# stwerner97/model-based-pde-control

Measured on AMD Instinct MI355X. Metric: KS sub-steps/sec (batched env), higher is better.
Workload: dtype f64

## Files before the change

model-based-pde-control_amd/csrc/fno.hip:

```cpp
#include <hip/hip_runtime.h>

#include <cstdio>
#include <map>
#include <mutex>
#include <utility>

#include "../../include/spectral/forward_select.h"
#include "../../include/spectral_hip.h"
#include "capi_error.h"

namespace {

typedef float f32x4 __attribute__((ext_vector_type(4)));

constexpr int C = 32;
constexpr int M = 16;
constexpr int K2 = 2 * M;
constexpr int KP = K2 + 4;
constexpr int KS = 2;
constexpr int TPB = 512;
constexpr int LAYERS = 4;

struct Weights {
    const float* lift_w;
// ... 27 lines not shown
    float cscale, cshift;
};

struct BwdArgs {
    Weights w;
    Rows u, act;
    const float* gdelta;
    const float* gout;
    int gout_t;
    const float* pre;
    float* gspec;
    float* rows;
    float* dbase;
    float* dact;
    const float* tabg;
    int n, nb, pairs;
    int spec_pairs, spec_pair0;
    float cscale;
};

constexpr int R_LIFT_W = 0, R_LIFT_B = 64, R_LAYER = 96, R_LAYER_SZ = 1024 + 32;
constexpr int R_P1W = R_LAYER + LAYERS * R_LAYER_SZ, R_P1B = R_P1W + 1024, R_P2W = R_P1B + 32, R_P2B = R_P2W + 32;
constexpr int ROW = ((R_P2B + 1 + 63) / 64) * 64;

__device__ __forceinline__ void gelu_parts(float x, float& cdf, float& pdf) {
    const float ax = fabsf(x);
    const float e = __expf(-0.5f * x * x);
    const float t = __frcp_rn(fmaf(0.3275911f * 0.70710678118654752f, ax, 1.0f));
    float poly = fmaf(1.061405429f, t, -1.453152027f);
    poly = fmaf(poly, t, 1.421413741f);
    poly = fmaf(poly, t, -0.284496736f);
    poly = fmaf(poly, t, 0.254829592f);
    const float erf_abs = fmaf(-poly * t, e, 1.0f);
    cdf = 0.5f * (1.0f + copysignf(erf_abs, x));
    pdf = 0.3989422804014327f * e;
}
__device__ __forceinline__ float gelu(float x) {
    float cdf, pdf;
    gelu_parts(x, cdf, pdf);
    return x * cdf;
}
__device__ __forceinline__ float gelu_grad(float x) {
    float cdf, pdf;
    gelu_parts(x, cdf, pdf);
    return fmaf(x, pdf, cdf);
}

#ifdef FNO_STAMP
__device__ unsigned long long g_stamps[256];
#define STAMP(k)                                                                      \
    do {                                                                              \
        if (blockIdx.x == 0 && threadIdx.x == 0) g_stamps[(k)] = __builtin_amdgcn_s_memtime(); \
    } while (0)
#else
#define STAMP(k) do { } while (0)
#endif

struct Lds {
    float *xs, *tb, *S, *Z, *wps, *gv, *misc;
    int NP;
    __device__ Lds(float* base, int N) {
        NP = N + 4;
        xs = base;
        tb = xs + C * NP;
        S = tb + C * NP;
        Z = S + KS * C * KP;
        wps = Z + C * KP;
        gv = wps + C * KP;
        misc = gv + N;
    }
    static size_t floats(int N) { return 2 * (size_t)C * (N + 4) + (KS + 2) * C * KP + (size_t)N + 256; }
};

__global__ void twiddle_init_kernel(float* tab, int N) {
    const int i = blockIdx.x * blockDim.x + threadIdx.x;
    if (i >= K2 * N) return;
    const int k = i / N, n = i - k * N;
    const bool is_sin = k >= M;
    const int mode = is_sin ? k - M : k;
    const int idx = (int)(((long)mode * n) % N);
    const float ang = 2.0f * (float)idx / (float)N;
    tab[i] = is_sin ? -sinpif(ang) : cospif(ang);
}
__device__ __forceinline__ void load_table(float* tab, const float* __restrict__ tabg, int N, int NP) {
    const int sh = __ffs(N) - 1;
    for (int i = threadIdx.x; i < (K2 * N) >> 2; i += blockDim.x) {
        const int e = i << 2, k = e >> sh, n = e & (N - 1);
        *reinterpret_cast<float4*>(tab + k * NP + n) = reinterpret_cast<const float4*>(tabg)[i];
    }
}

__device__ __forceinline__ void contract_n(const float* arows, const float* brows, float* S, int N, int NP) {
    const int lane = threadIdx.x & 63, wave = threadIdx.x >> 6, nwaves = blockDim.x >> 6;
    const int r = lane & 15, q = lane >> 4;
    for (int t = wave; t < 4 * KS; t += nwaves) {
        const int tile = t & 3, ks = t >> 2, rt = tile >> 1, ct = tile & 1;
        const int span = N / KS, kbeg = ks * span;
        const float* arow = arows + (16 * rt + r) * NP + kbeg;
        const float* brow = brows + (16 * ct + r) * NP + kbeg;
        f32x4 acc0 = {0.f, 0.f, 0.f, 0.f}, acc1 = {0.f, 0.f, 0.f, 0.f}, acc2 = {0.f, 0.f, 0.f, 0.f}, acc3 = {0.f, 0.f, 0.f, 0.f};
        for (int k0 = 0; k0 < span; k0 += 16) {
            const float a0 = arow[k0 + q], a1 = arow[k0 + 4 + q], a2 = arow[k0 + 8 + q], a3 = arow[k0 + 12 + q];
            const float b0 = brow[k0 + q], b1 = brow[k0 + 4 + q], b2 = brow[k0 + 8 + q], b3 = brow[k0 + 12 + q];
            acc0 = __builtin_amdgcn_mfma_f32_16x16x4f32(a0, b0, acc0, 0, 0, 0);
            acc1 = __builtin_amdgcn_mfma_f32_16x16x4f32(a1, b1, acc1, 0, 0, 0);
            acc2 = __builtin_amdgcn_mfma_f32_16x16x4f32(a2, b2, acc2, 0, 0, 0);
            acc3 = __builtin_amdgcn_mfma_f32_16x16x4f32(a3, b3, acc3, 0, 0, 0);
        }
        float* dst = S + ks * C * KP;
#pragma unroll
        for (int j = 0; j < 4; ++j) dst[(16 * rt + 4 * q + j) * KP + 16 * ct + r] = (acc0[j] + acc1[j]) + (acc2[j] + acc3[j]);
    }
}

__device__ __forceinline__ float s_sum(const float* S, int idx) {
    float v = S[idx];
#pragma unroll
    for (int ks = 1; ks < KS; ++ks) v += S[ks * C * KP + idx];
    return v;
}

__device__ __forceinline__ void load_mat(float* dst, const float* src) {
    for (int i = threadIdx.x; i < C * C; i += blockDim.x) dst[(i >> 5) * KP + (i & 31)] = src[i];
}

__device__ __forceinline__ void lift_into(float* xs, const float* u, const float* act, const Weights& w, int N, int NP) {
    const int sh = __ffs(N) - 1;
    for (int i = threadIdx.x; i < C * N; i += blockDim.x) {
        const int c = i >> sh, n = i & (N - 1);
        xs[c * NP + n] = fmaf(w.lift_w[2 * c], u[n], fmaf(w.lift_w[2 * c + 1], act[n], w.lift_b[c]));
    }
}

struct MixRegs {
    float4 vr[8], vi[8];
};
template <bool CONJ>
__device__ __forceinline__ void mix_load(const float* __restrict__ wr, const float* __restrict__ wi, MixRegs& m) {
    const int t = threadIdx.x, q4 = t & 3, m4 = (t >> 2) & 3, row = t >> 4;
#pragma unroll
    for (int c8 = 0; c8 < 8; ++c8) {
        const int c = 8 * q4 + c8;
        const size_t widx = CONJ ? ((size_t)row * C + c) * M + 4 * m4 : ((size_t)c * C + row) * M + 4 * m4;
        m.vr[c8] = *reinterpret_cast<const float4*>(wr + widx);
        m.vi[c8] = *reinterpret_cast<const float4*>(wi + widx);
    }
}
template <bool CONJ>
__device__ __forceinline__ void mix_compute(const MixRegs& w, const float* in, float* out, float s0, float s1) {
    const int t = threadIdx.x, q4 = t & 3, m4 = (t >> 2) & 3, row = t >> 4;
    float yr[4] = {0.f, 0.f, 0.f, 0.f}, yi[4] = {0.f, 0.f, 0.f, 0.f};
#pragma unroll
    for (int c8 = 0; c8 < 8; ++c8) {
        const int c = 8 * q4 + c8;
        float xr[4], xi[4];
#pragma unroll
        for (int j = 0; j < 4; ++j) {
            const int m = 4 * m4 + j;
            xr[j] = CONJ ? in[c * KP + m] : s_sum(in, c * KP + m);
            xi[j] = CONJ ? in[c * KP + M + m] : s_sum(in, c * KP + M + m);
        }
        const float wrv[4] = {w.vr[c8].x, w.vr[c8].y, w.vr[c8].z, w.vr[c8].w};
        const float wiv[4] = {w.vi[c8].x, w.vi[c8].y, w.vi[c8].z, w.vi[c8].w};
#pragma unroll
        for (int j = 0; j < 4; ++j) {
            if (CONJ) {
                yr[j] = fmaf(xr[j], wrv[j], fmaf(xi[j], wiv[j], yr[j]));
                yi[j] = fmaf(xi[j], wrv[j], fmaf(-xr[j], wiv[j], yi[j]));
            } else {
                yr[j] = fmaf(xr[j], wrv[j], fmaf(-xi[j], wiv[j], yr[j]));
                yi[j] = fmaf(xr[j], wiv[j], fmaf(xi[j], wrv[j], yi[j]));
            }
        }
    }
#pragma unroll
    for (int j = 0; j < 4; ++j) {
        yr[j] += __shfl_xor(yr[j], 1, 64);
        yi[j] += __shfl_xor(yi[j], 1, 64);
        yr[j] += __shfl_xor(yr[j], 2, 64);
        yi[j] += __shfl_xor(yi[j], 2, 64);
    }
    if (q4 == 0) {
#pragma unroll
        for (int j = 0; j < 4; ++j) {
            const int m = 4 * m4 + j;
            const float s = m == 0 ? s0 : s1;
            out[row * KP + m] = s * yr[j];
            out[row * KP + M + m] = s * yi[j];
        }
    }
}

template <bool SAVE>
__global__ void __launch_bounds__(TPB) fno_forward_kernel(const FwdArgs a) {
    extern __shared__ __align__(16) float lds_raw[];
    const int N = a.n;
    const Lds L(lds_raw, N);
    const int NP = L.NP;
    const int p = blockIdx.x, t = p / a.nb, b = p - t * a.nb;
    const int lane = threadIdx.x & 63, wave = threadIdx.x >> 6, nwaves = blockDim.x >> 6;
    const int r = lane & 15, q = lane >> 4;
    const float* u = a.u.row(t, b);
    const float* act = a.act.row(t, b);

    STAMP(0);
    lift_into(L.xs, u, act, a.w, N, NP);
    STAMP(1);
    load_table(L.tb, a.tabg, N, NP);
    __syncthreads();
    STAMP(2);

    const float s0 = 1.0f / (float)N, s1 = 2.0f / (float)N;
    for (int l = 0; l < LAYERS; ++l) {
        STAMP(3 + 4 * l);
        MixRegs mw;
        mix_load<false>(a.w.wr[l], a.w.wi[l], mw);
        contract_n(L.xs, L.tb, L.S, N, NP);
        load_mat(L.wps, a.w.pw[l]);
        if (threadIdx.x < C) L.misc[threadIdx.x] = a.w.pb[l][threadIdx.x];
        __syncthreads();
        STAMP(4 + 4 * l);
        if (SAVE) {
            for (int i = threadIdx.x; i < C * K2; i += blockDim.x) {
                const int k = i >> 5, c = i & 31;
                a.xspec[(((size_t)l * K2 + k) * a.spec_pairs + a.spec_pair0 + p) * C + c] = s_sum(L.S, c * KP + k);
            }
        }
        mix_compute<false>(mw, L.S, L.Z, s0, s1);
        __syncthreads();
        STAMP(5 + 4 * l);
        float* pre_out = SAVE ? a.pre + ((size_t)p * LAYERS + l) * C * N : nullptr;
        for (int ct = wave; ct < (N >> 4); ct += nwaves) {
            const int pos = 16 * ct + r;
            f32x4 acc[2][2];
#pragma unroll
            for (int rt = 0; rt < 2; ++rt) {
                acc[rt][0] = f32x4{0.f, 0.f, 0.f, 0.f};
                acc[rt][1] = f32x4{0.f, 0.f, 0.f, 0.f};
                const float* zrow = L.Z + (16 * rt + r) * KP;
                const float* wrow = L.wps + (16 * rt + r) * KP;
#pragma unroll
                for (int k0 = 0; k0 < K2; k0 += 4) {
                    acc[rt][0] = __builtin_amdgcn_mfma_f32_16x16x4f32(zrow[k0 + q], L.tb[(k0 + q) * NP + pos], acc[rt][0], 0, 0, 0);
                    acc[rt][1] = __builtin_amdgcn_mfma_f32_16x16x4f32(wrow[k0 + q], L.xs[(k0 + q) * NP + pos], acc[rt][1], 0, 0, 0);
                }
            }
#pragma unroll
            for (int rt = 0; rt < 2; ++rt)
#pragma unroll
                for (int j = 0; j < 4; ++j) {
                    const int row = 16 * rt + 4 * q + j;
                    const float v = (acc[rt][0][j] + acc[rt][1][j]) + L.misc[row];
                    if (SAVE) pre_out[(size_t)row * N + pos] = v;
                    L.xs[row * NP + pos] = l + 1 < LAYERS ? gelu(v) : v;
                }
        }
        __syncthreads();
        STAMP(6 + 4 * l);
    }

    STAMP(19);
    load_mat(L.wps, a.w.p1_w);
    if (threadIdx.x < C) {
        L.misc[threadIdx.x] = a.w.p1_b[threadIdx.x];
        L.misc[C + threadIdx.x] = a.w.p2_w[threadIdx.x];
    }
    __syncthreads();
    const float b2 = a.w.p2_b[0];
    for (int ct = wave; ct < (N >> 4); ct += nwaves) {
        const int pos = 16 * ct + r;
        float part = 0.0f;
#pragma unroll
        for (int rt = 0; rt < 2; ++rt) {
            f32x4 acc = {0.f, 0.f, 0.f, 0.f};
            const float* wrow = L.wps + (16 * rt + r) * KP;
#pragma unroll
            for (int k0 = 0; k0 < C; k0 += 4)
                acc = __builtin_amdgcn_mfma_f32_16x16x4f32(wrow[k0 + q], L.xs[(k0 + q) * NP + pos], acc, 0, 0, 0);
#pragma unroll
            for (int j = 0; j < 4; ++j) {
                const int row = 16 * rt + 4 * q + j;
                part = fmaf(L.misc[C + row], gelu(acc[j] + L.misc[row]), part);
            }
        }
        part += __shfl_xor(part, 16, 64);
        part += __shfl_xor(part, 32, 64);
        if (q == 0) {
            const float d = part + b2;
            a.delta[(size_t)p * N + pos] = d;
            if (a.out) a.out[(size_t)p * N + pos] = fmaf(a.cscale, d, u[pos]) + a.cshift;
        }
    }
    STAMP(20);
}

struct SelectArgs {
    Weights w[FNO_MAX_MEMBERS];
    float cscale[FNO_MAX_MEMBERS], cshift[FNO_MAX_MEMBERS];
    const int* chosen;
    const int* step;
    const float* u;
    const float* act;
    float* out;
    const float* tabg;
    int members, T, n, nb;
};

__global__ void __launch_bounds__(TPB) fno_forward_select_kernel(const SelectArgs a) {
    extern __shared__ __align__(16) float lds_raw[];
    const int N = a.n;
    const int b = blockIdx.x;
    const int t = a.step ? __builtin_amdgcn_readfirstlane(a.step[0]) : 0;
    if (t < 0 || t >= a.T) return;
    const int pick = a.chosen ? __builtin_amdgcn_readfirstlane(a.chosen[(long)t * a.nb + b]) : 0;
    float* out = a.out + (size_t)b * N;
    if (pick < 0 || pick >= a.members) {
        for (int n = threadIdx.x; n < N; n += blockDim.x) out[n] = NAN;
        return;
    }
    const Weights& w = a.w[pick];
    const float cscale = a.cscale[pick], cshift = a.cshift[pick];
    const Lds L(lds_raw, N);
    const int NP = L.NP;
    const int lane = threadIdx.x & 63, wave = threadIdx.x >> 6, nwaves = blockDim.x >> 6;
    const int r = lane & 15, q = lane >> 4;
    const float* u = a.u + (size_t)b * N;
    const float* act = a.act + (size_t)b * N;

    lift_into(L.xs, u, act, w, N, NP);
    load_table(L.tb, a.tabg, N, NP);
    __syncthreads();

    const float s0 = 1.0f / (float)N, s1 = 2.0f / (float)N;
    for (int l = 0; l < LAYERS; ++l) {
        MixRegs mw;
        mix_load<false>(w.wr[l], w.wi[l], mw);
        contract_n(L.xs, L.tb, L.S, N, NP);
        load_mat(L.wps, w.pw[l]);
        if (threadIdx.x < C) L.misc[threadIdx.x] = w.pb[l][threadIdx.x];
        __syncthreads();
        mix_compute<false>(mw, L.S, L.Z, s0, s1);
        __syncthreads();
        for (int ct = wave; ct < (N >> 4); ct += nwaves) {
            const int pos = 16 * ct + r;
            f32x4 acc[2][2];
#pragma unroll
            for (int rt = 0; rt < 2; ++rt) {
                acc[rt][0] = f32x4{0.f, 0.f, 0.f, 0.f};
                acc[rt][1] = f32x4{0.f, 0.f, 0.f, 0.f};
                const float* zrow = L.Z + (16 * rt + r) * KP;
                const float* wrow = L.wps + (16 * rt + r) * KP;
#pragma unroll
                for (int k0 = 0; k0 < K2; k0 += 4) {
                    acc[rt][0] = __builtin_amdgcn_mfma_f32_16x16x4f32(zrow[k0 + q], L.tb[(k0 + q) * NP + pos], acc[rt][0], 0, 0, 0);
                    acc[rt][1] = __builtin_amdgcn_mfma_f32_16x16x4f32(wrow[k0 + q], L.xs[(k0 + q) * NP + pos], acc[rt][1], 0, 0, 0);
                }
            }
#pragma unroll
            for (int rt = 0; rt < 2; ++rt)
#pragma unroll
                for (int j = 0; j < 4; ++j) {
                    const int row = 16 * rt + 4 * q + j;
                    const float v = (acc[rt][0][j] + acc[rt][1][j]) + L.misc[row];
                    L.xs[row * NP + pos] = l + 1 < LAYERS ? gelu(v) : v;
                }
        }
        __syncthreads();
    }

    load_mat(L.wps, w.p1_w);
    if (threadIdx.x < C) {
        L.misc[threadIdx.x] = w.p1_b[threadIdx.x];
        L.misc[C + threadIdx.x] = w.p2_w[threadIdx.x];
    }
    __syncthreads();
    const float b2 = w.p2_b[0];
    for (int ct = wave; ct < (N >> 4); ct += nwaves) {
        const int pos = 16 * ct + r;
        float part = 0.0f;
#pragma unroll
        for (int rt = 0; rt < 2; ++rt) {
            f32x4 acc = {0.f, 0.f, 0.f, 0.f};
            const float* wrow = L.wps + (16 * rt + r) * KP;
#pragma unroll
            for (int k0 = 0; k0 < C; k0 += 4)
                acc = __builtin_amdgcn_mfma_f32_16x16x4f32(wrow[k0 + q], L.xs[(k0 + q) * NP + pos], acc, 0, 0, 0);
#pragma unroll
            for (int j = 0; j < 4; ++j) {
                const int row = 16 * rt + 4 * q + j;
                part = fmaf(L.misc[C + row], gelu(acc[j] + L.misc[row]), part);
            }
        }
        part += __shfl_xor(part, 16, 64);
        part += __shfl_xor(part, 32, 64);
        if (q == 0) {
            const float d = part + b2;
            out[pos] = fmaf(cscale, d, u[pos]) + cshift;
        }
    }
}

__device__ __forceinline__ float row_dot(const float* buf, const float* v, int N, int NP) {
    const int row = threadIdx.x >> 4, l16 = threadIdx.x & 15;
    float s = 0.0f;
    if (row < C) {
        const float* src = buf + row * NP;
        if (v) {
            for (int n = l16; n < N; n += 16) s = fmaf(src[n], v[n], s);
        } else {
            for (int n = l16; n < N; n += 16) s += src[n];
        }
    }
    s += __shfl_xor(s, 1, 64);
    s += __shfl_xor(s, 2, 64);
    s += __shfl_xor(s, 4, 64);
    s += __shfl_xor(s, 8, 64);
    return s;
}

__global__ void __launch_bounds__(TPB) fno_backward_kernel(const BwdArgs a) {
    extern __shared__ __align__(16) float lds_raw[];
    const int N = a.n;
    const Lds L(lds_raw, N);
    const int NP = L.NP;
    float* db = L.tb;
    const int p = blockIdx.x, t = p / a.nb, b = p - t * a.nb;
    const int lane = threadIdx.x & 63, wave = threadIdx.x >> 6, nwaves = blockDim.x >> 6;
    const int r = lane & 15, q = lane >> 4;
    const int sh = __ffs(N) - 1;
    const float* u = a.u.row(t, b);
    const float* act = a.act.row(t, b);
    float* grow = a.rows + (size_t)p * ROW;
    const float* pre_p = a.pre + (size_t)p * LAYERS * C * N;
    const bool has_gout = a.gout && t == a.gout_t;

    for (int n = threadIdx.x; n < N; n += blockDim.x) {
        float g = a.gdelta[(size_t)p * N + n];
        if (has_gout) g = fmaf(a.cscale, a.gout[(size_t)b * N + n], g);
        L.gv[n] = g;
    }
    {
        const float4* src = reinterpret_cast<const float4*>(pre_p + (size_t)(LAYERS - 1) * C * N);
        for (int i = threadIdx.x; i < (C * N) >> 2; i += blockDim.x) {
            const int e = i << 2, c = e >> sh, n = e & (N - 1);
            *reinterpret_cast<float4*>(L.xs + c * NP + n) = src[i];
        }
    }
    load_mat(L.wps, a.w.p1_w);
    if (threadIdx.x < C) {
        L.misc[threadIdx.x] = a.w.p1_b[threadIdx.x];
        L.misc[C + threadIdx.x] = a.w.p2_w[threadIdx.x];
    }
    __syncthreads();

    {
        float dw2[2][4] = {{0.f, 0.f, 0.f, 0.f}, {0.f, 0.f, 0.f, 0.f}};
        for (int ct = wave; ct < (N >> 4); ct += nwaves) {
            const int pos = 16 * ct + r;
            const float g = L.gv[pos];
#pragma unroll
            for (int rt = 0; rt < 2; ++rt) {
                f32x4 acc = {0.f, 0.f, 0.f, 0.f};
                const float* wrow = L.wps + (16 * rt + r) * KP;
#pragma unroll
                for (int k0 = 0; k0 < C; k0 += 4)
                    acc = __builtin_amdgcn_mfma_f32_16x16x4f32(wrow[k0 + q], L.xs[(k0 + q) * NP + pos], acc, 0, 0, 0);
#pragma unroll
                for (int j = 0; j < 4; ++j) {
                    const int row = 16 * rt + 4 * q + j;
                    const float z1 = acc[j] + L.misc[row];
                    dw2[rt][j] = fmaf(g, gelu(z1), dw2[rt][j]);
                    db[row * NP + pos] = L.misc[C + row] * g * gelu_grad(z1);
                }
            }
        }
#pragma unroll
        for (int rt = 0; rt < 2; ++rt)
#pragma unroll
            for (int j = 0; j < 4; ++j) {
                float v = dw2[rt][j];
                v += __shfl_xor(v, 1, 64);
                v += __shfl_xor(v, 2, 64);
                v += __shfl_xor(v, 4, 64);
                v += __shfl_xor(v, 8, 64);
                if (r == 0) L.Z[wave * C + 16 * rt + 4 * q + j] = v;
            }
    }
    __syncthreads();
    contract_n(db, L.xs, L.S, N, NP);
    {
        const float s = row_dot(db, nullptr, N, NP);
        if ((threadIdx.x & 15) == 0 && (threadIdx.x >> 4) < C) grow[R_P1B + (threadIdx.x >> 4)] = s;
        if (threadIdx.x < C) {
            float v = L.Z[threadIdx.x];
            for (int w = 1; w < TPB / 64; ++w) v += L.Z[w * C + threadIdx.x];
            grow[R_P2W + threadIdx.x] = v;
        }
        if (wave == 0) {
            float g = 0.0f;
            for (int n = lane; n < N; n += 64) g += L.gv[n];
#pragma unroll
            for (int m = 1; m < 64; m <<= 1) g += __shfl_xor(g, m, 64);
            if (lane == 0) grow[R_P2B] = g;
        }
    }
    __syncthreads();
    for (int i = threadIdx.x; i < C * C; i += blockDim.x) grow[R_P1W + i] = s_sum(L.S, (i >> 5) * KP + (i & 31));
    for (int ct = wave; ct < (N >> 4); ct += nwaves) {
        const int pos = 16 * ct + r;
        f32x4 acc[2];
#pragma unroll
        for (int rt = 0; rt < 2; ++rt) {
            acc[rt] = f32x4{0.f, 0.f, 0.f, 0.f};
#pragma unroll
            for (int k0 = 0; k0 < C; k0 += 4)
                acc[rt] = __builtin_amdgcn_mfma_f32_16x16x4f32(L.wps[(k0 + q) * KP + 16 * rt + r], db[(k0 + q) * NP + pos], acc[rt], 0, 0, 0);
        }
#pragma unroll
        for (int rt = 0; rt < 2; ++rt)
#pragma unroll
            for (int j = 0; j < 4; ++j) db[(16 * rt + 4 * q + j) * NP + pos] = acc[rt][j];
    }
    __syncthreads();

    const float s0 = 1.0f / (float)N, s1 = 2.0f / (float)N;
    for (int l = LAYERS - 1; l >= 0; --l) {
        if (l + 1 < LAYERS) {
            const float4* src = reinterpret_cast<const float4*>(pre_p + (size_t)l * C * N);
            for (int i = threadIdx.x; i < (C * N) >> 2; i += blockDim.x) {
                const int e = i << 2, c = e >> sh, n = e & (N - 1);
                const float4 v = src[i];
                float4* d = reinterpret_cast<float4*>(db + c * NP + n);
                float4 g = *d;
                g.x *= gelu_grad(v.x);
                g.y *= gelu_grad(v.y);
                g.z *= gelu_grad(v.z);
                g.w *= gelu_grad(v.w);
                *d = g;
            }
        }
        if (l > 0) {
            const float4* src = reinterpret_cast<const float4*>(pre_p + (size_t)(l - 1) * C * N);
            for (int i = threadIdx.x; i < (C * N) >> 2; i += blockDim.x) {
                const int e = i << 2, c = e >> sh, n = e & (N - 1);
                float4 v = src[i];
                v.x = gelu(v.x);
                v.y = gelu(v.y);
                v.z = gelu(v.z);
                v.w = gelu(v.w);
                *reinterpret_cast<float4*>(L.xs + c * NP + n) = v;
            }
        } else {
            lift_into(L.xs, u, act, a.w, N, NP);
        }
        load_mat(L.wps, a.w.pw[l]);
        __syncthreads();
        contract_n(db, L.xs, L.S, N, NP);
        {
            const float s = row_dot(db, nullptr, N, NP);
            if ((threadIdx.x & 15) == 0 && (threadIdx.x >> 4) < C) grow[R_LAYER + l * R_LAYER_SZ + 1024 + (threadIdx.x >> 4)] = s;
        }
        __syncthreads();
        for (int i = threadIdx.x; i < C * C; i += blockDim.x)
            grow[R_LAYER + l * R_LAYER_SZ + i] = s_sum(L.S, (i >> 5) * KP + (i & 31));
        load_table(L.xs, a.tabg, N, NP);
        __syncthreads();
        MixRegs mw;
        mix_load<true>(a.w.wr[l], a.w.wi[l], mw);
        contract_n(db, L.xs, L.S, N, NP);
        __syncthreads();
        for (int i = threadIdx.x; i < C * K2; i += blockDim.x) {
            const int k = i >> 5, c = i & 31, m = k & (M - 1);
            const float g = s_sum(L.S, c * KP + k) * (m == 0 ? s0 : s1);
            L.Z[c * KP + k] = g;
            a.gspec[(((size_t)l * K2 + k) * a.spec_pairs + a.spec_pair0 + p) * C + c] = g;
        }
        __syncthreads();
        mix_compute<true>(mw, L.Z, L.S, 1.0f, 1.0f);
        __syncthreads();
        for (int ct = wave; ct < (N >> 4); ct += nwaves) {
            const int pos = 16 * ct + r;
            f32x4 acc[2][2];
#pragma unroll
            for (int rt = 0; rt < 2; ++rt) {
                acc[rt][0] = f32x4{0.f, 0.f, 0.f, 0.f};
                acc[rt][1] = f32x4{0.f, 0.f, 0.f, 0.f};
                const float* zrow = L.S + (16 * rt + r) * KP;
#pragma unroll
                for (int k0 = 0; k0 < K2; k0 += 4) {
                    acc[rt][0] = __builtin_amdgcn_mfma_f32_16x16x4f32(zrow[k0 + q], L.xs[(k0 + q) * NP + pos], acc[rt][0], 0, 0, 0);
                    acc[rt][1] = __builtin_amdgcn_mfma_f32_16x16x4f32(L.wps[(k0 + q) * KP + 16 * rt + r], db[(k0 + q) * NP + pos], acc[rt][1], 0, 0, 0);
                }
            }
#pragma unroll
            for (int rt = 0; rt < 2; ++rt)
#pragma unroll
                for (int j = 0; j < 4; ++j) db[(16 * rt + 4 * q + j) * NP + pos] = acc[rt][0][j] + acc[rt][1][j];
        }
        __syncthreads();
    }

    for (int n = threadIdx.x; n < N; n += blockDim.x) {
        L.gv[n] = u[n];
        L.Z[n] = act[n];
    }
    if (threadIdx.x < C) {
        L.misc[threadIdx.x] = a.w.lift_w[2 * threadIdx.x];
        L.misc[C + threadIdx.x] = a.w.lift_w[2 * threadIdx.x + 1];
    }
    __syncthreads();
    {
        const float su = row_dot(db, L.gv, N, NP), sa = row_dot(db, L.Z, N, NP), sb = row_dot(db, nullptr, N, NP);
        if ((threadIdx.x & 15) == 0 && (threadIdx.x >> 4) < C) {
            const int c = threadIdx.x >> 4;
            grow[R_LIFT_W + 2 * c] = su;
            grow[R_LIFT_W + 2 * c + 1] = sa;
            grow[R_LIFT_B + c] = sb;
        }
    }
    if (a.dbase) {
        for (int n = threadIdx.x; n < N; n += blockDim.x) {
            float s = 0.0f;
#pragma unroll 8
            for (int c = 0; c < C; ++c) s = fmaf(L.misc[c], db[c * NP + n], s);
            if (has_gout) s += a.gout[(size_t)b * N + n];
            a.dbase[(size_t)p * N + n] = s;
        }
    }
    if (a.dact) {
        for (int n = threadIdx.x; n < N; n += blockDim.x) {
            float s = 0.0f;
#pragma unroll 8
            for (int c = 0; c < C; ++c) s = fmaf(L.misc[C + c], db[c * NP + n], s);
            a.dact[(size_t)p * N + n] = s;
        }
    }
}

__global__ void __launch_bounds__(512) fno_reduce_rows_kernel(const float* rows, int pairs, int width, float* out) {
    __shared__ float part[8][64];
    const int col = threadIdx.x & 63, grp = threadIdx.x >> 6;
    const int j = blockIdx.x * 64 + col;
    float s0 = 0.0f, s1 = 0.0f, s2 = 0.0f, s3 = 0.0f;
    if (j < width) {
        int p = grp;
        for (; p + 24 < pairs; p += 32) {
            s0 += rows[(size_t)p * width + j];
            s1 += rows[(size_t)(p + 8) * width + j];
            s2 += rows[(size_t)(p + 16) * width + j];
            s3 += rows[(size_t)(p + 24) * width + j];
        }
        for (; p < pairs; p += 8) s0 += rows[(size_t)p * width + j];
    }
    part[grp][col] = (s0 + s1) + (s2 + s3);
    __syncthreads();
    if (grp == 0 && j < width) {
        float v = part[0][col];
#pragma unroll
        for (int g = 1; g < 8; ++g) v += part[g][col];
        out[j] = v;
    }
}

struct WgradOut {
    float* dwr[LAYERS];
    float* dwi[LAYERS];
};

constexpr int WG_KS = 4;
__global__ void __launch_bounds__(256 * WG_KS) fno_spec_wgrad_kernel(const float* xspec, const float* gspec, int pairs, const WgradOut dst) {
    __shared__ float part[WG_KS][4][2][256];
    const int l = blockIdx.x / M, m = blockIdx.x % M;
    const int lane = threadIdx.x & 63, wave = threadIdx.x >> 6;
    const int tile = wave & 3, ks = wave >> 2;
    const int r = lane & 15, q = lane >> 4;
    const int rt = tile >> 1, ct = tile & 1;
    const size_t plane = (size_t)pairs * C;
    const float* xr = xspec + ((size_t)l * K2 + m) * plane;
    const float* xi = xspec + ((size_t)l * K2 + M + m) * plane;
    const float* gr = gspec + ((size_t)l * K2 + m) * plane;
    const float* gi = gspec + ((size_t)l * K2 + M + m) * plane;
    f32x4 rr = {0.f, 0.f, 0.f, 0.f}, ii = {0.f, 0.f, 0.f, 0.f}, ir = {0.f, 0.f, 0.f, 0.f}, ri = {0.f, 0.f, 0.f, 0.f};
    for (int p0 = 4 * ks; p0 < pairs; p0 += 4 * WG_KS) {
        const int pp = p0 + q;
        const bool ok = pp < pairs;
        const size_t row = (size_t)(ok ? pp : 0) * C;
        const float axr = ok ? xr[row + 16 * rt + r] : 0.f, axi = ok ? xi[row + 16 * rt + r] : 0.f;
        const float bgr = ok ? gr[row + 16 * ct + r] : 0.f, bgi = ok ? gi[row + 16 * ct + r] : 0.f;
        rr = __builtin_amdgcn_mfma_f32_16x16x4f32(axr, bgr, rr, 0, 0, 0);
        ii = __builtin_amdgcn_mfma_f32_16x16x4f32(axi, bgi, ii, 0, 0, 0);
        ir = __builtin_amdgcn_mfma_f32_16x16x4f32(axr, bgi, ir, 0, 0, 0);
        ri = __builtin_amdgcn_mfma_f32_16x16x4f32(axi, bgr, ri, 0, 0, 0);
    }
#pragma unroll
    for (int j = 0; j < 4; ++j) {
        part[ks][tile][0][lane * 4 + j] = rr[j] + ii[j];
        part[ks][tile][1][lane * 4 + j] = ir[j] - ri[j];
    }
    __syncthreads();
    if (ks == 0) {
        float* outr = dst.dwr[l];
        float* outi = dst.dwi[l];
#pragma unroll
        for (int j = 0; j < 4; ++j) {
            float vr = part[0][tile][0][lane * 4 + j], vi = part[0][tile][1][lane * 4 + j];
#pragma unroll
            for (int k = 1; k < WG_KS; ++k) {
                vr += part[k][tile][0][lane * 4 + j];
                vi += part[k][tile][1][lane * 4 + j];
            }
            const int i = 16 * rt + 4 * q + j, o = 16 * ct + r;
            const size_t idx = ((size_t)i * C + o) * M + m;
            outr[idx] = vr;
            outi[idx] = vi;
        }
    }
}

int check(const char* who, int n, int nb, int pairs, int width, int modes, int layers) {
// ... 200 lines not shown
```

Before: 1.366 billion.

## Restructure FNO kernels with register-held MFMA tiles, software-pipelined contraction, prefetched loads

After: 1.363 billion. Within noise of the previous version (-0.2%).

```diff
diff --git a/model-based-pde-control_amd/csrc/fno.hip b/model-based-pde-control_amd/csrc/fno.hip
--- a/model-based-pde-control_amd/csrc/fno.hip
+++ b/model-based-pde-control_amd/csrc/fno.hip
@@ -133,12 +133,26 @@
     const float ang = 2.0f * (float)idx / (float)N;
     tab[i] = is_sin ? -sinpif(ang) : cospif(ang);
 }
-__device__ __forceinline__ void load_table(float* tab, const float* __restrict__ tabg, int N, int NP) {
+struct Block8 {
+    float4 v[8];
+};
+__device__ __forceinline__ void block_issue(Block8& b, const float* __restrict__ src, int N) {
+#pragma unroll
+    for (int j = 0; j < 8; ++j)
+        b.v[j] = j * TPB < (C * N) >> 2 ? reinterpret_cast<const float4*>(src)[j * TPB + threadIdx.x] : float4{0.f, 0.f, 0.f, 0.f};
+}
+template <typename F>
+__device__ __forceinline__ void block_each(const Block8& b, int N, int NP, F f) {
     const int sh = __ffs(N) - 1;
-    for (int i = threadIdx.x; i < (K2 * N) >> 2; i += blockDim.x) {
-        const int e = i << 2, k = e >> sh, n = e & (N - 1);
-        *reinterpret_cast<float4*>(tab + k * NP + n) = reinterpret_cast<const float4*>(tabg)[i];
-    }
+#pragma unroll
+    for (int j = 0; j < 8; ++j)
+        if (j * TPB < (C * N) >> 2) {
+            const int e = (j * TPB + threadIdx.x) << 2;
+            f(b.v[j], (e >> sh) * NP + (e & (N - 1)));
+        }
+}
+__device__ __forceinline__ void store_table(float* tab, const Block8& b, int N, int NP) {
+    block_each(b, N, NP, [&](const float4& v, int at) { *reinterpret_cast<float4*>(tab + at) = v; });
 }
 
 __device__ __forceinline__ void contract_n(const float* arows, const float* brows, float* S, int N, int NP) {
@@ -147,17 +161,28 @@
     for (int t = wave; t < 4 * KS; t += nwaves) {
         const int tile = t & 3, ks = t >> 2, rt = tile >> 1, ct = tile & 1;
         const int span = N / KS, kbeg = ks * span;
-        const float* arow = arows + (16 * rt + r) * NP + kbeg;
-        const float* brow = brows + (16 * ct + r) * NP + kbeg;
+        const float4* arow = reinterpret_cast<const float4*>(arows + (16 * rt + r) * NP + kbeg + 4 * q);
+        const float4* brow = reinterpret_cast<const float4*>(brows + (16 * ct + r) * NP + kbeg + 4 * q);
         f32x4 acc0 = {0.f, 0.f, 0.f, 0.f}, acc1 = {0.f, 0.f, 0.f, 0.f}, acc2 = {0.f, 0.f, 0.f, 0.f}, acc3 = {0.f, 0.f, 0.f, 0.f};
-        for (int k0 = 0; k0 < span; k0 += 16) {
-            const float a0 = arow[k0 + q], a1 = arow[k0 + 4 + q], a2 = arow[k0 + 8 + q], a3 = arow[k0 + 12 + q];
-            const float b0 = brow[k0 + q], b1 = brow[k0 + 4 + q], b2 = brow[k0 + 8 + q], b3 = brow[k0 + 12 + q];
-            acc0 = __builtin_amdgcn_mfma_f32_16x16x4f32(a0, b0, acc0, 0, 0, 0);
-            acc1 = __builtin_amdgcn_mfma_f32_16x16x4f32(a1, b1, acc1, 0, 0, 0);
-            acc2 = __builtin_amdgcn_mfma_f32_16x16x4f32(a2, b2, acc2, 0, 0, 0);
-            acc3 = __builtin_amdgcn_mfma_f32_16x16x4f32(a3, b3, acc3, 0, 0, 0);
-        }
+        float4 a0 = arow[0], b0 = brow[0], a1 = arow[4], b1 = brow[4];
+        auto round = [&](const float4& xa, const float4& xb, const float4& ya, const float4& yb) {
+            acc0 = __builtin_amdgcn_mfma_f32_16x16x4f32(xa.x, xb.x, acc0, 0, 0, 0);
+            acc1 = __builtin_amdgcn_mfma_f32_16x16x4f32(xa.y, xb.y, acc1, 0, 0, 0);
+            acc2 = __builtin_amdgcn_mfma_f32_16x16x4f32(xa.z, xb.z, acc2, 0, 0, 0);
+            acc3 = __builtin_amdgcn_mfma_f32_16x16x4f32(xa.w, xb.w, acc3, 0, 0, 0);
+            acc0 = __builtin_amdgcn_mfma_f32_16x16x4f32(ya.x, yb.x, acc0, 0, 0, 0);
+            acc1 = __builtin_amdgcn_mfma_f32_16x16x4f32(ya.y, yb.y, acc1, 0, 0, 0);
+            acc2 = __builtin_amdgcn_mfma_f32_16x16x4f32(ya.z, yb.z, acc2, 0, 0, 0);
+            acc3 = __builtin_amdgcn_mfma_f32_16x16x4f32(ya.w, yb.w, acc3, 0, 0, 0);
+        };
+        for (int k4 = 8; k4 < span >> 2; k4 += 8) {
+            const float4 na0 = arow[k4], nb0 = brow[k4], na1 = arow[k4 + 4], nb1 = brow[k4 + 4];
+            __builtin_amdgcn_sched_barrier(0);
+            round(a0, b0, a1, b1);
+            __builtin_amdgcn_sched_barrier(0);
+            a0 = na0, b0 = nb0, a1 = na1, b1 = nb1;
+        }
+        round(a0, b0, a1, b1);
         float* dst = S + ks * C * KP;
 #pragma unroll
         for (int j = 0; j < 4; ++j) dst[(16 * rt + 4 * q + j) * KP + 16 * ct + r] = (acc0[j] + acc1[j]) + (acc2[j] + acc3[j]);
@@ -171,16 +196,24 @@
     return v;
 }
 
+__device__ __forceinline__ void fold_spectrum(float* S, float* xspec, size_t kstride) {
+    for (int i = threadIdx.x; i < C * K2; i += blockDim.x) {
+        const int k = xspec ? i >> 5 : i & 31, c = xspec ? i & 31 : i >> 5;
+        const float v = s_sum(S, c * KP + k);
+        S[c * KP + k] = v;
+        if (xspec) xspec[k * kstride + c] = v;
+    }
+}
+
 __device__ __forceinline__ void load_mat(float* dst, const float* src) {
     for (int i = threadIdx.x; i < C * C; i += blockDim.x) dst[(i >> 5) * KP + (i & 31)] = src[i];
 }
 
 __device__ __forceinline__ void lift_into(float* xs, const float* u, const float* act, const Weights& w, int N, int NP) {
     const int sh = __ffs(N) - 1;
-    for (int i = threadIdx.x; i < C * N; i += blockDim.x) {
-        const int c = i >> sh, n = i & (N - 1);
-        xs[c * NP + n] = fmaf(w.lift_w[2 * c], u[n], fmaf(w.lift_w[2 * c + 1], act[n], w.lift_b[c]));
-    }
+    const int n = threadIdx.x & (N - 1), g = threadIdx.x >> sh, ng = blockDim.x >> sh;
+    const float un = u[n], an = act[n];
+    for (int c = g; c < C; c += ng) xs[c * NP + n] = fmaf(w.lift_w[2 * c], un, fmaf(w.lift_w[2 * c + 1], an, w.lift_b[c]));
 }
 
 struct MixRegs {
@@ -204,13 +237,9 @@
 #pragma unroll
     for (int c8 = 0; c8 < 8; ++c8) {
         const int c = 8 * q4 + c8;
-        float xr[4], xi[4];
-#pragma unroll
-        for (int j = 0; j < 4; ++j) {
-            const int m = 4 * m4 + j;
-            xr[j] = CONJ ? in[c * KP + m] : s_sum(in, c * KP + m);
-            xi[j] = CONJ ? in[c * KP + M + m] : s_sum(in, c * KP + M + m);
-        }
+        const float4 x4r = *reinterpret_cast<const float4*>(in + c * KP + 4 * m4);
+        const float4 x4i = *reinterpret_cast<const float4*>(in + c * KP + M + 4 * m4);
+        const float xr[4] = {x4r.x, x4r.y, x4r.z, x4r.w}, xi[4] = {x4i.x, x4i.y, x4i.z, x4i.w};
         const float wrv[4] = {w.vr[c8].x, w.vr[c8].y, w.vr[c8].z, w.vr[c8].w};
         const float wiv[4] = {w.vi[c8].x, w.vi[c8].y, w.vi[c8].z, w.vi[c8].w};
 #pragma unroll
@@ -242,6 +271,94 @@
     }
 }
 
+struct ATiles {
+    float v[2][8];
+};
+template <bool TRANS>
+__device__ __forceinline__ ATiles load_a(const float* mat, int r, int q) {
+    ATiles a;
+#pragma unroll
+    for (int rt = 0; rt < 2; ++rt)
+#pragma unroll
+        for (int j = 0; j < 8; ++j) a.v[rt][j] = TRANS ? mat[(4 * j + q) * KP + 16 * rt + r] : mat[(16 * rt + r) * KP + 4 * j + q];
+    return a;
+}
+struct BCol {
+    float v[8];
+};
+__device__ __forceinline__ void load_b(BCol& b, const float* buf, int NP, int pos, int q) {
+#pragma unroll
+    for (int j = 0; j < 8; ++j) b.v[j] = buf[(4 * j + q) * NP + pos];
+}
+__device__ __forceinline__ void tile_mfma(f32x4 (&acc)[2], const ATiles& a, const BCol& b) {
+#pragma unroll
+    for (int j = 0; j < 8; ++j) {
+        acc[0] = __builtin_amdgcn_mfma_f32_16x16x4f32(a.v[0][j], b.v[j], acc[0], 0, 0, 0);
+        acc[1] = __builtin_amdgcn_mfma_f32_16x16x4f32(a.v[1][j], b.v[j], acc[1], 0, 0, 0);
+    }
+}
+
+__device__ __forceinline__ void layer_tiles(const Lds& L, int N, bool activate, float* pre_out) {
+    const int lane = threadIdx.x & 63, wave = threadIdx.x >> 6, nwaves = blockDim.x >> 6;
+    const int r = lane & 15, q = lane >> 4, NP = L.NP, tiles = N >> 4;
+    if (wave >= tiles) return;
+    const ATiles za = load_a<false>(L.Z, r, q), wa = load_a<false>(L.wps, r, q);
+    float bias[2][4];
+#pragma unroll
+    for (int rt = 0; rt < 2; ++rt)
+#pragma unroll
+        for (int j = 0; j < 4; ++j) bias[rt][j] = L.misc[16 * rt + 4 * q + j];
+    for (int ct = wave; ct < tiles; ct += nwaves) {
+        const int pos = 16 * ct + r;
+        BCol bt, bx;
+        load_b(bt, L.tb, NP, pos, q);
+        load_b(bx, L.xs, NP, pos, q);
+        f32x4 az[2] = {{0.f, 0.f, 0.f, 0.f}, {0.f, 0.f, 0.f, 0.f}}, aw[2] = {{0.f, 0.f, 0.f, 0.f}, {0.f, 0.f, 0.f, 0.f}};
+        tile_mfma(az, za, bt);
+        tile_mfma(aw, wa, bx);
+#pragma unroll
+        for (int rt = 0; rt < 2; ++rt)
+#pragma unroll
+            for (int j = 0; j < 4; ++j) {
+                const int row = 16 * rt + 4 * q + j;
+                const float v = (az[rt][j] + aw[rt][j]) + bias[rt][j];
+                if (pre_out) pre_out[(size_t)row * N + pos] = v;
+                L.xs[row * NP + pos] = activate ? gelu(v) : v;
+            }
+    }
+}
+
+template <typename Emit>
+__device__ __forceinline__ void project_tiles(const Lds& L, int N, float b2, Emit emit) {
+    const int lane = threadIdx.x & 63, wave = threadIdx.x >> 6, nwaves = blockDim.x >> 6;
+    const int r = lane & 15, q = lane >> 4, NP = L.NP, tiles = N >> 4;
+    if (wave >= tiles) return;
+    const ATiles wa = load_a<false>(L.wps, r, q);
+    float b1[2][4], w2[2][4];
+#pragma unroll
+    for (int rt = 0; rt < 2; ++rt)
+#pragma unroll
+        for (int j = 0; j < 4; ++j) {
+            b1[rt][j] = L.misc[16 * rt + 4 * q + j];
+            w2[rt][j] = L.misc[C + 16 * rt + 4 * q + j];
+        }
+    for (int ct = wave; ct < tiles; ct += nwaves) {
+        const int pos = 16 * ct + r;
+        BCol bx;
+        load_b(bx, L.xs, NP, pos, q);
+        f32x4 acc[2] = {{0.f, 0.f, 0.f, 0.f}, {0.f, 0.f, 0.f, 0.f}};
+        tile_mfma(acc, wa, bx);
+        float part = 0.0f;
+#pragma unroll
+        for (int rt = 0; rt < 2; ++rt)
+#pragma unroll
+            for (int j = 0; j < 4; ++j) part = fmaf(w2[rt][j], gelu(acc[rt][j] + b1[rt][j]), part);
+        part += __shfl_xor(part, 16, 64);
+        part += __shfl_xor(part, 32, 64);
+        if (q == 0) emit(pos, part + b2);
+    }
+}
+
 template <bool SAVE>
 __global__ void __launch_bounds__(TPB) fno_forward_kernel(const FwdArgs a) {
     extern __shared__ __align__(16) float lds_raw[];
@@ -249,63 +366,37 @@
     const Lds L(lds_raw, N);
     const int NP = L.NP;
     const int p = blockIdx.x, t = p / a.nb, b = p - t * a.nb;
-    const int lane = threadIdx.x & 63, wave = threadIdx.x >> 6, nwaves = blockDim.x >> 6;
-    const int r = lane & 15, q = lane >> 4;
     const float* u = a.u.row(t, b);
     const float* act = a.act.row(t, b);
 
     STAMP(0);
     lift_into(L.xs, u, act, a.w, N, NP);
     STAMP(1);
-    load_table(L.tb, a.tabg, N, NP);
+    {
+        Block8 tab;
+        block_issue(tab, a.tabg, N);
+        store_table(L.tb, tab, N, NP);
+    }
     __syncthreads();
     STAMP(2);
 
+    MixRegs mw;
     const float s0 = 1.0f / (float)N, s1 = 2.0f / (float)N;
     for (int l = 0; l < LAYERS; ++l) {
         STAMP(3 + 4 * l);
-        MixRegs mw;
-        mix_load<false>(a.w.wr[l], a.w.wi[l], mw);
+        if (l == 0) mix_load<false>(a.w.wr[0], a.w.wi[0], mw);
         contract_n(L.xs, L.tb, L.S, N, NP);
         load_mat(L.wps, a.w.pw[l]);
         if (threadIdx.x < C) L.misc[threadIdx.x] = a.w.pb[l][threadIdx.x];
         __syncthreads();
         STAMP(4 + 4 * l);
-        if (SAVE) {
-            for (int i = threadIdx.x; i < C * K2; i += blockDim.x) {
-                const int k = i >> 5, c = i & 31;
-                a.xspec[(((size_t)l * K2 + k) * a.spec_pairs + a.spec_pair0 + p) * C + c] = s_sum(L.S, c * KP + k);
-            }
-        }
+        fold_spectrum(L.S, SAVE ? a.xspec + ((size_t)l * K2 * a.spec_pairs + a.spec_pair0 + p) * C : nullptr, (size_t)a.spec_pairs * C);
+        __syncthreads();
         mix_compute<false>(mw, L.S, L.Z, s0, s1);
+        if (l + 1 < LAYERS) mix_load<false>(a.w.wr[l + 1], a.w.wi[l + 1], mw);
         __syncthreads();
         STAMP(5 + 4 * l);
-        float* pre_out = SAVE ? a.pre + ((size_t)p * LAYERS + l) * C * N : nullptr;
-        for (int ct = wave; ct < (N >> 4); ct += nwaves) {
-            const int pos = 16 * ct + r;
-            f32x4 acc[2][2];
-#pragma unroll
-            for (int rt = 0; rt < 2; ++rt) {
-                acc[rt][0] = f32x4{0.f, 0.f, 0.f, 0.f};
-                acc[rt][1] = f32x4{0.f, 0.f, 0.f, 0.f};
-                const float* zrow = L.Z + (16 * rt + r) * KP;
-                const float* wrow = L.wps + (16 * rt + r) * KP;
-#pragma unroll
-                for (int k0 = 0; k0 < K2; k0 += 4) {
-                    acc[rt][0] = __builtin_amdgcn_mfma_f32_16x16x4f32(zrow[k0 + q], L.tb[(k0 + q) * NP + pos], acc[rt][0], 0, 0, 0);
-                    acc[rt][1] = __builtin_amdgcn_mfma_f32_16x16x4f32(wrow[k0 + q], L.xs[(k0 + q) * NP + pos], acc[rt][1], 0, 0, 0);
-                }
-            }
-#pragma unroll
-            for (int rt = 0; rt < 2; ++rt)
-#pragma unroll
-                for (int j = 0; j < 4; ++j) {
-                    const int row = 16 * rt + 4 * q + j;
-                    const float v = (acc[rt][0][j] + acc[rt][1][j]) + L.misc[row];
-                    if (SAVE) pre_out[(size_t)row * N + pos] = v;
-                    L.xs[row * NP + pos] = l + 1 < LAYERS ? gelu(v) : v;
-                }
-        }
+        layer_tiles(L, N, l + 1 < LAYERS, SAVE ? a.pre + ((size_t)p * LAYERS + l) * C * N : nullptr);
         __syncthreads();
         STAMP(6 + 4 * l);
     }
@@ -317,31 +408,10 @@
         L.misc[C + threadIdx.x] = a.w.p2_w[threadIdx.x];
     }
     __syncthreads();
-    const float b2 = a.w.p2_b[0];
-    for (int ct = wave; ct < (N >> 4); ct += nwaves) {
-        const int pos = 16 * ct + r;
-        float part = 0.0f;
-#pragma unroll
-        for (int rt = 0; rt < 2; ++rt) {
-            f32x4 acc = {0.f, 0.f, 0.f, 0.f};
-            const float* wrow = L.wps + (16 * rt + r) * KP;
-#pragma unroll
-            for (int k0 = 0; k0 < C; k0 += 4)
-                acc = __builtin_amdgcn_mfma_f32_16x16x4f32(wrow[k0 + q], L.xs[(k0 + q) * NP + pos], acc, 0, 0, 0);
-#pragma unroll
-            for (int j = 0; j < 4; ++j) {
-                const int row = 16 * rt + 4 * q + j;
-                part = fmaf(L.misc[C + row], gelu(acc[j] + L.misc[row]), part);
-            }
-        }
-        part += __shfl_xor(part, 16, 64);
-        part += __shfl_xor(part, 32, 64);
-        if (q == 0) {
-            const float d = part + b2;
-            a.delta[(size_t)p * N + pos] = d;
-            if (a.out) a.out[(size_t)p * N + pos] = fmaf(a.cscale, d, u[pos]) + a.cshift;
-        }
-    }
+    project_tiles(L, N, a.w.p2_b[0], [&](int pos, float d) {
+        a.delta[(size_t)p * N + pos] = d;
+        if (a.out) a.out[(size_t)p * N + pos] = fmaf(a.cscale, d, u[pos]) + a.cshift;
+    });
     STAMP(20);
 }
 
@@ -373,49 +443,31 @@
     const float cscale = a.cscale[pick], cshift = a.cshift[pick];
     const Lds L(lds_raw, N);
     const int NP = L.NP;
-    const int lane = threadIdx.x & 63, wave = threadIdx.x >> 6, nwaves = blockDim.x >> 6;
-    const int r = lane & 15, q = lane >> 4;
     const float* u = a.u + (size_t)b * N;
     const float* act = a.act + (size_t)b * N;
 
     lift_into(L.xs, u, act, w, N, NP);
-    load_table(L.tb, a.tabg, N, NP);
+    {
+        Block8 tab;
+        block_issue(tab, a.tabg, N);
+        store_table(L.tb, tab, N, NP);
+    }
     __syncthreads();
 
+    MixRegs mw;
     const float s0 = 1.0f / (float)N, s1 = 2.0f / (float)N;
     for (int l = 0; l < LAYERS; ++l) {
-        MixRegs mw;
-        mix_load<false>(w.wr[l], w.wi[l], mw);
+        if (l == 0) mix_load<false>(w.wr[0], w.wi[0], mw);
         contract_n(L.xs, L.tb, L.S, N, NP);
         load_mat(L.wps, w.pw[l]);
         if (threadIdx.x < C) L.misc[threadIdx.x] = w.pb[l][threadIdx.x];
         __syncthreads();
+        fold_spectrum(L.S, nullptr, 0);
+        __syncthreads();
         mix_compute<false>(mw, L.S, L.Z, s0, s1);
-        __syncthreads();
-        for (int ct = wave; ct < (N >> 4); ct += nwaves) {
-            const int pos = 16 * ct + r;
-            f32x4 acc[2][2];
-#pragma unroll
-            for (int rt = 0; rt < 2; ++rt) {
-                acc[rt][0] = f32x4{0.f, 0.f, 0.f, 0.f};
-                acc[rt][1] = f32x4{0.f, 0.f, 0.f, 0.f};
-                const float* zrow = L.Z + (16 * rt + r) * KP;
-                const float* wrow = L.wps + (16 * rt + r) * KP;
-#pragma unroll
-                for (int k0 = 0; k0 < K2; k0 += 4) {
-                    acc[rt][0] = __builtin_amdgcn_mfma_f32_16x16x4f32(zrow[k0 + q], L.tb[(k0 + q) * NP + pos], acc[rt][0], 0, 0, 0);
-                    acc[rt][1] = __builtin_amdgcn_mfma_f32_16x16x4f32(wrow[k0 + q], L.xs[(k0 + q) * NP + pos], acc[rt][1], 0, 0, 0);
-                }
-            }
-#pragma unroll
-            for (int rt = 0; rt < 2; ++rt)
-#pragma unroll
-                for (int j = 0; j < 4; ++j) {
-                    const int row = 16 * rt + 4 * q + j;
-                    const float v = (acc[rt][0][j] + acc[rt][1][j]) + L.misc[row];
-                    L.xs[row * NP + pos] = l + 1 < LAYERS ? gelu(v) : v;
-                }
-        }
+        if (l + 1 < LAYERS) mix_load<false>(w.wr[l + 1], w.wi[l + 1], mw);
+        __syncthreads();
+        layer_tiles(L, N, l + 1 < LAYERS, nullptr);
         __syncthreads();
     }
 
@@ -425,30 +477,7 @@
         L.misc[C + threadIdx.x] = w.p2_w[threadIdx.x];
     }
     __syncthreads();
-    const float b2 = w.p2_b[0];
-    for (int ct = wave; ct < (N >> 4); ct += nwaves) {
-        const int pos = 16 * ct + r;
-        float part = 0.0f;
-#pragma unroll
-        for (int rt = 0; rt < 2; ++rt) {
-            f32x4 acc = {0.f, 0.f, 0.f, 0.f};
-            const float* wrow = L.wps + (16 * rt + r) * KP;
-#pragma unroll
-            for (int k0 = 0; k0 < C; k0 += 4)
-                acc = __builtin_amdgcn_mfma_f32_16x16x4f32(wrow[k0 + q], L.xs[(k0 + q) * NP + pos], acc, 0, 0, 0);
-#pragma unroll
-            for (int j = 0; j < 4; ++j) {
-                const int row = 16 * rt + 4 * q + j;
-                part = fmaf(L.misc[C + row], gelu(acc[j] + L.misc[row]), part);
-            }
-        }
-        part += __shfl_xor(part, 16, 64);
-        part += __shfl_xor(part, 32, 64);
-        if (q == 0) {
-            const float d = part + b2;
-            out[pos] = fmaf(cscale, d, u[pos]) + cshift;
-        }
-    }
+    project_tiles(L, N, w.p2_b[0], [&](int pos, float d) { out[pos] = fmaf(cscale, d, u[pos]) + cshift; });
 }
 
 __device__ __forceinline__ float row_dot(const float* buf, const float* v, int N, int NP) {
@@ -478,24 +507,23 @@
     const int p = blockIdx.x, t = p / a.nb, b = p - t * a.nb;
     const int lane = threadIdx.x & 63, wave = threadIdx.x >> 6, nwaves = blockDim.x >> 6;
     const int r = lane & 15, q = lane >> 4;
-    const int sh = __ffs(N) - 1;
+    const int tiles = N >> 4;
     const float* u = a.u.row(t, b);
     const float* act = a.act.row(t, b);
     float* grow = a.rows + (size_t)p * ROW;
     const float* pre_p = a.pre + (size_t)p * LAYERS * C * N;
     const bool has_gout = a.gout && t == a.gout_t;
 
+    STAMP(32);
     for (int n = threadIdx.x; n < N; n += blockDim.x) {
         float g = a.gdelta[(size_t)p * N + n];
         if (has_gout) g = fmaf(a.cscale, a.gout[(size_t)b * N + n], g);
         L.gv[n] = g;
     }
     {
-        const float4* src = reinterpret_cast<const float4*>(pre_p + (size_t)(LAYERS - 1) * C * N);
-        for (int i = threadIdx.x; i < (C * N) >> 2; i += blockDim.x) {
-            const int e = i << 2, c = e >> sh, n = e & (N - 1);
-            *reinterpret_cast<float4*>(L.xs + c * NP + n) = src[i];
-        }
+        Block8 h;
+        block_issue(h, pre_p + (size_t)(LAYERS - 1) * C * N, N);
+        block_each(h, N, NP, [&](const float4& v, int at) { *reinterpret_cast<float4*>(L.xs + at) = v; });
     }
     load_mat(L.wps, a.w.p1_w);
     if (threadIdx.x < C) {
@@ -506,23 +534,31 @@
 
     {
         float dw2[2][4] = {{0.f, 0.f, 0.f, 0.f}, {0.f, 0.f, 0.f, 0.f}};
-        for (int ct = wave; ct < (N >> 4); ct += nwaves) {
-            const int pos = 16 * ct + r;
-            const float g = L.gv[pos];
-#pragma unroll
-            for (int rt = 0; rt < 2; ++rt) {
-                f32x4 acc = {0.f, 0.f, 0.f, 0.f};
-                const float* wrow = L.wps + (16 * rt + r) * KP;
-#pragma unroll
-                for (int k0 = 0; k0 < C; k0 += 4)
-                    acc = __builtin_amdgcn_mfma_f32_16x16x4f32(wrow[k0 + q], L.xs[(k0 + q) * NP + pos], acc, 0, 0, 0);
+        if (wave < tiles) {
+            const ATiles wa = load_a<false>(L.wps, r, q);
+            float b1[2][4], w2[2][4];
+#pragma unroll
+            for (int rt = 0; rt < 2; ++rt)
 #pragma unroll
                 for (int j = 0; j < 4; ++j) {
-                    const int row = 16 * rt + 4 * q + j;
-                    const float z1 = acc[j] + L.misc[row];
-                    dw2[rt][j] = fmaf(g, gelu(z1), dw2[rt][j]);
-                    db[row * NP + pos] = L.misc[C + row] * g * gelu_grad(z1);
+                    b1[rt][j] = L.misc[16 * rt + 4 * q + j];
+                    w2[rt][j] = L.misc[C + 16 * rt + 4 * q + j];
                 }
+            for (int ct = wave; ct < tiles; ct += nwaves) {
+                const int pos = 16 * ct + r;
+                const float g = L.gv[pos];
+                BCol bx;
+                load_b(bx, L.xs, NP, pos, q);
+                f32x4 acc[2] = {{0.f, 0.f, 0.f, 0.f}, {0.f, 0.f, 0.f, 0.f}};
+                tile_mfma(acc, wa, bx);
+#pragma unroll
+                for (int rt = 0; rt < 2; ++rt)
+#pragma unroll
+                    for (int j = 0; j < 4; ++j) {
+                        const float z1 = acc[rt][j] + b1[rt][j];
+                        dw2[rt][j] = fmaf(g, gelu(z1), dw2[rt][j]);
+                        db[(16 * rt + 4 * q + j) * NP + pos] = w2[rt][j] * g * gelu_grad(z1);
+                    }
             }
         }
 #pragma unroll
@@ -557,69 +593,72 @@
     }
     __syncthreads();
     for (int i = threadIdx.x; i < C * C; i += blockDim.x) grow[R_P1W + i] = s_sum(L.S, (i >> 5) * KP + (i & 31));
-    for (int ct = wave; ct < (N >> 4); ct += nwaves) {
-        const int pos = 16 * ct + r;
-        f32x4 acc[2];
-#pragma unroll
-        for (int rt = 0; rt < 2; ++rt) {
-            acc[rt] = f32x4{0.f, 0.f, 0.f, 0.f};
-#pragma unroll
-            for (int k0 = 0; k0 < C; k0 += 4)
-                acc[rt] = __builtin_amdgcn_mfma_f32_16x16x4f32(L.wps[(k0 + q) * KP + 16 * rt + r], db[(k0 + q) * NP + pos], acc[rt], 0, 0, 0);
-        }
-#pragma unroll
-        for (int rt = 0; rt < 2; ++rt)
-#pragma unroll
-            for (int j = 0; j < 4; ++j) db[(16 * rt + 4 * q + j) * NP + pos] = acc[rt][j];
+    if (wave < tiles) {
+        const ATiles wa = load_a<true>(L.wps, r, q);
+        for (int ct = wave; ct < tiles; ct += nwaves) {
+            const int pos = 16 * ct + r;
+            BCol bd;
+            load_b(bd, db, NP, pos, q);
+            f32x4 acc[2] = {{0.f, 0.f, 0.f, 0.f}, {0.f, 0.f, 0.f, 0.f}};
+            tile_mfma(acc, wa, bd);
+#pragma unroll
+            for (int rt = 0; rt < 2; ++rt)
+#pragma unroll
+                for (int j = 0; j < 4; ++j) db[(16 * rt + 4 * q + j) * NP + pos] = acc[rt][j];
+        }
     }
     __syncthreads();
+    STAMP(33);
 
     const float s0 = 1.0f / (float)N, s1 = 2.0f / (float)N;
     for (int l = LAYERS - 1; l >= 0; --l) {
+        STAMP(40 + 8 * l);
+        Block8 pl, px;
         if (l + 1 < LAYERS) {
-            const float4* src = reinterpret_cast<const float4*>(pre_p + (size_t)l * C * N);
-            for (int i = threadIdx.x; i < (C * N) >> 2; i += blockDim.x) {
-                const int e = i << 2, c = e >> sh, n = e & (N - 1);
-                const float4 v = src[i];
-                float4* d = reinterpret_cast<float4*>(db + c * NP + n);
+            block_issue(pl, pre_p + (size_t)l * C * N, N);
+            block_each(pl, N, NP, [&](const float4& v, int at) {
+                float4* d = reinterpret_cast<float4*>(db + at);
                 float4 g = *d;
                 g.x *= gelu_grad(v.x);
                 g.y *= gelu_grad(v.y);
                 g.z *= gelu_grad(v.z);
                 g.w *= gelu_grad(v.w);
                 *d = g;
-            }
+            });
         }
         if (l > 0) {
-            const float4* src = reinterpret_cast<const float4*>(pre_p + (size_t)(l - 1) * C * N);
-            for (int i = threadIdx.x; i < (C * N) >> 2; i += blockDim.x) {
-                const int e = i << 2, c = e >> sh, n = e & (N - 1);
-                float4 v = src[i];
+            block_issue(px, pre_p + (size_t)(l - 1) * C * N, N);
+            block_each(px, N, NP, [&](float4 v, int at) {
                 v.x = gelu(v.x);
                 v.y = gelu(v.y);
                 v.z = gelu(v.z);
                 v.w = gelu(v.w);
-                *reinterpret_cast<float4*>(L.xs + c * NP + n) = v;
-            }
+                *reinterpret_cast<float4*>(L.xs + at) = v;
+            });
         } else {
             lift_into(L.xs, u, act, a.w, N, NP);
         }
         load_mat(L.wps, a.w.pw[l]);
         __syncthreads();
+        STAMP(41 + 8 * l);
         contract_n(db, L.xs, L.S, N, NP);
         {
             const float s = row_dot(db, nullptr, N, NP);
             if ((threadIdx.x & 15) == 0 && (threadIdx.x >> 4) < C) grow[R_LAYER + l * R_LAYER_SZ + 1024 + (threadIdx.x >> 4)] = s;
         }
         __syncthreads();
+        Block8 tab;
+        block_issue(tab, a.tabg, N);
         for (int i = threadIdx.x; i < C * C; i += blockDim.x)
             grow[R_LAYER + l * R_LAYER_SZ + i] = s_sum(L.S, (i >> 5) * KP + (i & 31));
-        load_table(L.xs, a.tabg, N, NP);
-        __syncthreads();
+        store_table(L.xs, tab, N, NP);
+        __syncthreads();
+        STAMP(42 + 8 * l);
         MixRegs mw;
         mix_load<true>(a.w.wr[l], a.w.wi[l], mw);
         contract_n(db, L.xs, L.S, N, NP);
         __syncthreads();
+        STAMP(43 + 8 * l);
         for (int i = threadIdx.x; i < C * K2; i += blockDim.x) {
             const int k = i >> 5, c = i & 31, m = k & (M - 1);
             const float g = s_sum(L.S, c * KP + k) * (m == 0 ? s0 : s1);
@@ -629,26 +668,25 @@
         __syncthreads();
         mix_compute<true>(mw, L.Z, L.S, 1.0f, 1.0f);
         __syncthreads();
-        for (int ct = wave; ct < (N >> 4); ct += nwaves) {
-            const int pos = 16 * ct + r;
-            f32x4 acc[2][2];
-#pragma unroll
-            for (int rt = 0; rt < 2; ++rt) {
-                acc[rt][0] = f32x4{0.f, 0.f, 0.f, 0.f};
-                acc[rt][1] = f32x4{0.f, 0.f, 0.f, 0.f};
-                const float* zrow = L.S + (16 * rt + r) * KP;
-#pragma unroll
-                for (int k0 = 0; k0 < K2; k0 += 4) {
-                    acc[rt][0] = __builtin_amdgcn_mfma_f32_16x16x4f32(zrow[k0 + q], L.xs[(k0 + q) * NP + pos], acc[rt][0], 0, 0, 0);
-                    acc[rt][1] = __builtin_amdgcn_mfma_f32_16x16x4f32(L.wps[(k0 + q) * KP + 16 * rt + r], db[(k0 + q) * NP + pos], acc[rt][1], 0, 0, 0);
-                }
+        STAMP(44 + 8 * l);
+        if (wave < tiles) {
+            const ATiles za = load_a<false>(L.S, r, q), wa = load_a<true>(L.wps, r, q);
+            for (int ct = wave; ct < tiles; ct += nwaves) {
+                const int pos = 16 * ct + r;
+                BCol bt, bd;
+                load_b(bt, L.xs, NP, pos, q);
+                load_b(bd, db, NP, pos, q);
+                f32x4 az[2] = {{0.f, 0.f, 0.f, 0.f}, {0.f, 0.f, 0.f, 0.f}}, aw[2] = {{0.f, 0.f, 0.f, 0.f}, {0.f, 0.f, 0.f, 0.f}};
+                tile_mfma(az, za, bt);
+                tile_mfma(aw, wa, bd);
+#pragma unroll
+                for (int rt = 0; rt < 2; ++rt)
+#pragma unroll
+                    for (int j = 0; j < 4; ++j) db[(16 * rt + 4 * q + j) * NP + pos] = az[rt][j] + aw[rt][j];
             }
-#pragma unroll
-            for (int rt = 0; rt < 2; ++rt)
-#pragma unroll
-                for (int j = 0; j < 4; ++j) db[(16 * rt + 4 * q + j) * NP + pos] = acc[rt][0][j] + acc[rt][1][j];
-        }
-        __syncthreads();
+        }
+        __syncthreads();
+        STAMP(45 + 8 * l);
     }
 
     for (int n = threadIdx.x; n < N; n += blockDim.x) {
@@ -686,6 +724,7 @@
             a.dact[(size_t)p * N + n] = s;
         }
     }
+    STAMP(80);
 }
 
 __global__ void __launch_bounds__(512) fno_reduce_rows_kernel(const float* rows, int pairs, int width, float* out) {
```
